# dronefreak/CABiNet

Measured on NVIDIA B200. Metric: images/sec at 1024x1024 (MNv3-L), higher is better.
Workload: dtype bf16

## Files before the change

cabinet_b200/_lib.py:

```python

from __future__ import annotations

import ctypes as C
import subprocess
from pathlib import Path

PKG = Path(__file__).resolve().parent
LIB_PATH = PKG / "libcabinet_b200.so"
CSRC = PKG / "csrc"

F32, BF16, F16 = 0, 1, 2
ACT_NONE, ACT_RELU, ACT_HSWISH, ACT_HSIGMOID, ACT_SIGMOID = 0, 1, 2, 3, 4

_p, _i, _ll, _f = C.c_void_p, C.c_int, C.c_longlong, C.c_float

SIGNATURES = {
    "cabinet_last_error": ([], C.c_char_p),
    "cabinet_abi_version": ([], _i),
    "cabinet_device_info": ([C.POINTER(_i)] * 3, _i),
    "cabinet_debug_flags": ([_i], _i),
    "cabinet_debug_read": ([_p, _i], _i),
    "cabinet_conv2d_simt": ([_p, _i, _ll, _ll, _ll, _ll, _ll, _p, _i, _ll, _ll, _ll, _p, _p, _ll, _p, _i, _ll, _ll,
                             _i, _i, _i, _i, _i, _i, _i, _i, _i, _i, _i, _i, _i, _f, _p], _i),
    "cabinet_conv_tc": ([_p, _ll, _i, _i, _i, _i, _p, _i, _i, _i, _i, _i, _p, _p, _ll, _p, _i, _ll, _i, _i, _i, _p], _i),
    "cabinet_conv_tc_dt": ([_p, _ll, _i, _i, _i, _i, _p, _i, _i, _i, _i, _i, _p, _p, _ll, _p, _i, _ll, _i, _i, _i, _i, _p],
                           _i),
    "cabinet_conv_tc_view": ([_p, _ll, _i, _i, _i, _i, _p, _i, _i, _i, _i, _p, _p, _ll, _i, _i, _ll, _ll, _ll, _p], _i),
    "cabinet_conv_tc_view_dt": ([_p, _ll, _i, _i, _i, _i, _p, _i, _i, _i, _i, _p, _p, _ll, _i, _i, _ll, _ll, _ll, _i, _p], _i),
    "cabinet_conv_tc_se": ([_p, _ll, _i, _i, _i, _i, _p, _i, _p, _i, _i, _i, _i, _i, _p, _p, _ll, _p, _i, _ll, _i, _i, _i,
                            _p], _i),
    "cabinet_conv_tc_split_act": ([_p, _ll, _i, _i, _i, _i, _p, _i, _i, _i, _i, _i, _p, _p, _i, _ll, _i, _i, _i, _i, _p], _i),
    "cabinet_conv_tc_imgw": ([_p, _ll, _i, _i, _i, _i, _p, _ll, _i, _i, _i, _i, _i, _p, _p, _ll, _p, _i, _ll, _i, _i, _i,
                              _p], _i),
    "cabinet_conv_tc_imgw_dt": ([_p, _ll, _i, _i, _i, _i, _p, _ll, _i, _i, _i, _i, _i, _p, _p, _ll, _p, _i, _ll, _i, _i, _i,
                                 _i, _p], _i),
    "cabinet_conv_tc_up": ([_p, _ll, _i, _i, _i, _i, _p, _i, _i, _i, _i, _i, _p, _p, _i, _i, _p, _ll, _i, _i, _i, _p], _i),
    "cabinet_gate_scale_weights": ([_p, _i, _f, _p, _p, _p, _p, _i, _i, _i, _p, _p, _i, _i, _i, _i, _i, _p], _i),
    "cabinet_scale_weights": ([_p, _p, _p, _i, _i, _i, _i, _i, _i, _p], _i),
    "cabinet_stem_tc": ([_p, _i, _i, _i, _p, _p, _p, _ll, _p, _ll, _i, _i, _p], _i),
    "cabinet_stem_tc2": ([_p, _i, _i, _i, _p, _p, _ll, _p, _ll, _i, _i, _p], _i),
    "cabinet_dwconv": ([_p, _ll, _p, _p, _p, _ll, _i, _i, _i, _i, _i, _i, _i, _i, _i, _i, _p, _p], _i),
    "cabinet_dwconv_tma": ([_p, _ll, _p, _p, _p, _ll, _i, _i, _i, _i, _i, _i, _i, _i, _i, _p, _p], _i),
    "cabinet_dwconv_tma_dt": ([_p, _ll, _p, _p, _p, _ll, _i, _i, _i, _i, _i, _i, _i, _i, _i, _p, _i, _p], _i),
    "cabinet_mbconv_noexpand_fused": ([_p, _ll, _p, _p, _p, _p, _p, _ll, _i, _i, _i, _i, _i, _p], _i),
    "cabinet_mbconv_fused": ([_p, _ll, _i, _i, _i, _i, _p, _p, _i, _i, _i, _i, _i, _p, _p, _i, _i, _p, _ll, _i, _i, _p,
                              _p], _i),
    "cabinet_mbconv_t": ([_p, _ll, _i, _i, _i, _i, _p, _p, _i, _i, _i, _i, _i, _p, _p, _i, _i, _p, _ll, _i, _i, _p, _p,
                          _p], _i),
    "cabinet_expand_sums": ([_p, _ll, _i, _i, _i, _i, _p, _p, _i, _i, _i, _i, _p, _p], _i),
    "cabinet_gate_mlp": ([_p, _f, _p, _p, _p, _p, _p, _i, _i, _i, _i, _p], _i),
    "cabinet_gate_fc": ([_p, _f, _p, _p, _p, _i, _i, _i, _i, _i, _p], _i),
    "cabinet_scale_act": ([_p, _ll, _i, _p, _i, _ll, _i, _i, _i, _p], _i),
    "cabinet_psp_pool": ([_p, _ll, _i, _p, _i, _i, _i, _i, _p, _ll, _p], _i),
    "cabinet_psp_concat": ([_p, _ll, _p, _p, _ll, _i, _i, _i, _i, _i, _p], _i),
    "cabinet_softmax_rows": ([_p, _p, _i, _ll, _i, _p], _i),
    "cabinet_attention_tc": ([_p, _ll, _p, _ll, _p, _ll, _p, _p, _ll, _i, _i, _i, _f, _p], _i),
    "cabinet_cab_combine": ([_p, _p, _p, _p, _ll, _p, _i, _ll, _i, _p], _i),
    "cabinet_channel_sum": ([_p, _ll, _i, _i, _ll, _i, _p, _p, _ll, _p], _i),
    "cabinet_bilinear_nhwc": ([_p, _ll, _i, _p, _ll, _i, _i, _i, _i, _i, _i, _i, _p], _i),
    "cabinet_upsample_logits_nchw": ([_p, _i, _i, _i, _i, _p, _i, _i, _i, _p], _i),
    "cabinet_upsample_argmax": ([_p, _i, _i, _i, _i, _p, _i, _i, _p, _i, _i, _p, _p], _i),
    "cabinet_normalize_u8": ([_p, _p, _i, _i, _i, _f, _f, _f, _f, _f, _f, _p], _i),
    "cabinet_confusion_hist": ([_p, _i, _p, _i, _ll, _i, _i, _p, _p], _i),
    "cabinet_upsample_softmax_accum": ([_p, _p, _i, _i, _i, _i, _i, _i, _p, _ll, _ll, _ll, _i, _i, _i, _i, _p, _p, _f,
                                        _p], _i),
    "cabinet_prob_resize_accum": ([_p, _i, _i, _i, _i, _i, _i, _i, _i, _p, _i, _i, _p], _i),
    "cabinet_argmax_hist_nchw": ([_p, _i, _i, _ll, _p, _p, _i, _i, _p, _p], _i),
    "cabinet_ohem_workspace_bytes": ([], _ll),
    "cabinet_train_scratch_floats": ([_ll, _i, _i], _ll),
    "cabinet_pack_conv_weight": ([_p, _i, _i, _i, _i, _p, _i, _i, _i, _i, _p], _i),
    "cabinet_pack_conv_weight_parity": ([_p, _i, _i, _i, _i, _i, _i, _i, _i, _i, _p, _i, _i, _p], _i),
    "cabinet_pack_conv_weight_parity_dt": ([_p, _i, _i, _i, _i, _i, _i, _i, _i, _i, _p, _i, _i, _i, _p], _i),
    "cabinet_pack_dw_weight": ([_p, _i, _i, _i, _p, _p], _i),
    "cabinet_im2col_nchw": ([_p, _i, _i, _i, _i, _i, _i, _i, _p, _ll, _p], _i),
    "cabinet_im2col_nchw_dt": ([_p, _i, _i, _i, _i, _i, _i, _i, _p, _ll, _i, _p], _i),
    "cabinet_embed_filter": ([_p, _i, _i, _i, _i, _p, _ll, _i, _p], _i),
    "cabinet_bn_train_stats": ([_p, _ll, _i, _ll, _i, _p, _p, _f, _f, _p, _p, _p, _p, _p], _i),
    "cabinet_affine_act": ([_p, _ll, _i, _p, _p, _p, _f, _p, _ll, _p, _ll, _i, _ll, _ll, _i, _i, _p], _i),
    "cabinet_bn_train_backward": ([_p, _ll, _p, _ll, _i, _p, _i, _p, _p, _p, _ll, _ll, _i, _i, _p, _p], _i),
    "cabinet_bn_frozen_stats": ([_p, _p, _p, _p, _f, _i, _p, _p], _i),
    "cabinet_bn_frozen_backward": ([_p, _ll, _p, _ll, _i, _p, _i, _p, _p, _p, _ll, _ll, _i, _i, _p, _p], _i),
    "cabinet_stem_dgrad": ([_p, _ll, _p, _ll, _i, _p, _p, _p, _i, _i, _i, _i, _i, _p], _i),
    "cabinet_gate_scale_backward": ([_p, _ll, _p, _ll, _i, _p, _f, _i, _p, _i, _ll, _i, _p, _p], _i),
    "cabinet_gate_apply_backward": ([_p, _ll, _p, _ll, _i, _p, _f, _p, _f, _i, _p, _ll, _i, _ll, _i, _i, _p], _i),
    "cabinet_gate_mlp_backward": ([_p, _f, _p, _p, _p, _p, _p, _i, _i, _i, _i, _p, _p, _p, _p, _p, _p, _p], _i),
    "cabinet_col_sum": ([_p, _ll, _i, _ll, _i, _p, _i, _p, _p], _i),
    "cabinet_conv_dgrad": ([_p, _ll, _i, _p, _i, _ll, _ll, _p, _ll, _i, _i, _i, _i, _i, _i, _i, _i, _i, _i, _i, _i, _p], _i),
    "cabinet_conv_wgrad_scratch_floats": ([_i, _i, _i, _i, _i, _i, _i], _ll),
    "cabinet_conv_wgrad": ([_p, _ll, _i, _p, _i, _ll, _ll, _ll, _ll, _p, _i, _i, _i, _i, _i, _i, _i, _i, _i, _i, _i, _p,
                            _p], _i),
    "cabinet_conv_wgrad_tc_scratch_floats": ([_i, _i, _i, _i, _i, _i, _i, _i, _i], _ll),
    "cabinet_conv_wgrad_tc": ([_p, _ll, _p, _ll, _p, _i, _i, _i, _i, _i, _i, _i, _i, _i, _p, _p], _i),
    "cabinet_conv_wgrad_tc_dt": ([_p, _ll, _p, _ll, _p, _i, _i, _i, _i, _i, _i, _i, _i, _i, _p, _i, _p], _i),
# ... 57 lines not shown
```

cabinet_b200/engine.py:

```python

from __future__ import annotations

import math
from dataclasses import dataclass
from typing import Optional

import torch

from . import _lib
from ._lib import ACT_HSIGMOID, ACT_HSWISH, ACT_NONE, ACT_RELU, ACT_SIGMOID, BF16, F16, F32, check
from .constants import BN_EPS


_DTYPE_CODES = {torch.float32: F32, torch.bfloat16: BF16, torch.float16: F16}


def dtype_code(dtype: torch.dtype) -> int:
    code = _DTYPE_CODES.get(dtype)
    if code is None:
        raise TypeError(f"cabinet_b200 kernels take float32, bfloat16 or float16 tensors, got {dtype}")
    return code


@dataclass
# ... 75 lines not shown

    def __init__(self, w1, b1, w2, b2, gate):
        f = lambda t: None if t is None else _host(t).reshape(t.shape[0], -1).contiguous()
        self.w1, self.w2 = f(w1), f(w2)
        self.b1 = None if b1 is None else _host(b1).contiguous()
        self.b2 = None if b2 is None else _host(b2).contiguous()
        self.cmid, self.c = self.w1.shape
        self.gate = gate


_LAYER_TYPES = {c.__name__: c for c in (ConvLayer, DwLayer, GateLayer)}


def _to_plain(o):
    if type(o).__name__ in _LAYER_TYPES:
        return {"__layer__": type(o).__name__, "vars": {k: _to_plain(v) for k, v in vars(o).items()}}
    if isinstance(o, dict):
        return {k: _to_plain(v) for k, v in o.items()}
    if isinstance(o, (list, tuple)):
        return type(o)(_to_plain(v) for v in o)
    return o


def _map_tensors(o, fn):
    if isinstance(o, torch.Tensor):
        return fn(o)
    if type(o).__name__ in _LAYER_TYPES:
        for k, v in vars(o).items():
            setattr(o, k, _map_tensors(v, fn))
        return o
    if isinstance(o, dict):
        return {k: _map_tensors(v, fn) for k, v in o.items()}
    if isinstance(o, (list, tuple)):
        return type(o)(_map_tensors(v, fn) for v in o)
    return o


def _from_plain(o):
    if isinstance(o, dict):
        if "__layer__" in o:
            obj = object.__new__(_LAYER_TYPES[o["__layer__"]])
            obj.__dict__.update({k: _from_plain(v) for k, v in o["vars"].items()})
            return obj
        return {k: _from_plain(v) for k, v in o.items()}
    if isinstance(o, (list, tuple)):
        return type(o)(_from_plain(v) for v in o)
    return o


def _out_size(n, k, s, p):
    return (n + 2 * p - k) // s + 1


class Engine:
    PACKED_ATTRS = ("stem", "blocks", "last", "stem_tc", "sb1", "sb2", "sb3", "sb4", "conva", "to_q", "to_k", "to_v",
                    "psp_k", "psp_v", "proj_out", "local", "gamma", "convb", "b1", "b4", "key_ch", "qkv", "ffm_blk",
                    "ffm_gate", "head_conv", "head_out", "ffm_sb", "low_fold", "stem_tc2")

    def __init__(self, model, precision: str = "bf16", packed: Optional[dict] = None):
        if precision not in ("bf16", "fp32"):
            raise ValueError(f"precision must be 'bf16' or 'fp32', got {precision!r}")
        p0 = next(model.parameters())
        if not p0.is_cuda:
            raise RuntimeError("cabinet_b200 engine needs the model on a CUDA device (no CPU path)")
        self.lib = _lib.load()
        self.dev = p0.device
        self.precision = precision
        self.tdt = torch.bfloat16 if precision == "bf16" else torch.float32
        self.dt = BF16 if precision == "bf16" else F32
        self.n_classes = model.n_classes
        self.stamp = None
        self.launches = 0
        self.use_tc = precision == "bf16"
        self.debug = False
        self.stages = {}
        self.trace, self.trace_filter = None, None
        self.fuse_mbconv = True
        self.se_from_sums = True
        self.use_stem2 = True
        self.t_small_s2 = False
        self.t_k5s2 = True
        self.use_mbconv_t = True
        self.fold_se_relu = True
        self.fold_ffm = True
        self.fold_low_up = False
        self.reverse_layers = frozenset()
        self.fuse_se = False
        self.fuse_se_blocks = frozenset({"mobile.f12", "mobile.f13"})
        self.use_cuda_graph = False
        self.sub_batch = 0
        self._graphs = {}
        self._pool = None
        self._graph_seen = {}
        self.dual_stream = False
        self._side = None
        self._scratch = []
        self.branch_overlap = True
        self._branch_streams, self._branch_events = [], {}
        self.sb_overlap = False
        if packed is not None:
            missing = [a for a in self.PACKED_ATTRS if a not in packed]
            if missing:
                raise ValueError(f"packed weights lack {missing}")
            for a in self.PACKED_ATTRS:
                setattr(self, a, _from_plain(packed[a]))
            self.gamma = model.ab.a2block.gamma.detach().float().contiguous()
        else:
            with torch.no_grad():
                self._pack(model)
                for a in self.PACKED_ATTRS:
                    setattr(self, a, _map_tensors(getattr(self, a), lambda t: t.to(self.dev)))

    def packed_state(self) -> dict:
        return {a: _to_plain(getattr(self, a)) for a in self.PACKED_ATTRS}

    def _pack(self, m):
        wd = self.tdt
        f32 = torch.float32
        mob = m.mobile
        self.stem = ConvLayer(mob.features[0][0], mob.features[0][1], ACT_HSWISH, f32, "mobile.stem")
        self.blocks = []
        for bi, blk in enumerate(list(mob.features)[1:], 1):
            s, c = blk.spec, blk.conv
            act = ACT_HSWISH if s["hs"] else ACT_RELU
            e = dict(spec=s, act=act)
            if s["expand"]:
                e["pw1"] = ConvLayer(c[0], c[1], act, wd, f"mobile.f{bi}.expand")
                e["dw"] = DwLayer(c[3], c[4], ACT_NONE if s["se"] else act, f"mobile.f{bi}.dw")
                se, pw2, bn2 = c[5], c[7], c[8]
                if self.precision == "bf16":
                    dwl, kk, nc = e["dw"], e["dw"].k ** 2, -(-e["dw"].c // 64)
                    aux = torch.zeros((nc * 64, kk + 2), dtype=f32, device=dwl.w.device)
# ... 1 lines not shown
                    aux[: dwl.c, kk + 1] = dwl.b
                    e["aux"] = aux.view(nc, 64, kk + 2).permute(0, 2, 1).contiguous()
                    p1 = e["pw1"]
                    if p1.cin % 8 == 0 and p1.cin % 64 <= 56 and p1.cin <= 248:
                        wb = torch.zeros((-(-p1.cout // 16) * 16, (p1.cin // 64 + 1) * 64), dtype=f32, device=dwl.w.device)
                        wb[: p1.cout, : p1.cin] = p1.tc[: p1.cout, 0, : p1.cin].float()
                        hi = p1.b.to(torch.bfloat16).float()
                        wb[: p1.cout, p1.cin], wb[: p1.cout, p1.cin + 1] = hi, p1.b - hi
                        e["w1b"] = wb.to(torch.bfloat16).contiguous()
                        ch = 64 if dwl.c <= 64 else 128
                        nct = 1 if dwl.c <= 64 else -(-dwl.c // 128)
                        flat = torch.zeros((nct * ch, wb.shape[1]), dtype=f32, device=dwl.w.device)
                        flat[: dwl.c] = wb[: dwl.c]
                        e["w1t"] = (flat.view(nct, ch, -1).repeat(1, 128 // ch, 1).reshape(nct * 128, -1)
                                    .to(torch.bfloat16).contiguous())
                        fa = torch.zeros((nct * ch, kk + 1), dtype=f32, device=dwl.w.device)
                        fa[: dwl.c, :kk] = dwl.w.t()
                        fa[: dwl.c, kk] = dwl.b
                        e["auxt"] = fa.view(nct, ch, kk + 1).repeat(1, 128 // ch, 1).permute(0, 2, 1).contiguous()
            else:
                e["dw"] = DwLayer(c[0], c[1], act, f"mobile.f{bi}.dw")
                se, pw2, bn2 = c[3], c[4], c[5]
            if s["se"]:
                e["se"] = GateLayer(se.fc[0].weight, se.fc[0].bias, se.fc[2].weight, se.fc[2].bias, ACT_HSIGMOID)
            e["pw2"] = ConvLayer(pw2, bn2, ACT_NONE, wd, f"mobile.f{bi}.project")
            if (not s["expand"] and not s["se"] and s["identity"] and s["k"] == 3 and s["exp"] in (8, 16, 32)
                    and self.precision == "bf16"):
                w2, b2 = _fold(pw2.weight, pw2.bias, bn2)
                e["fused_pw"] = (w2.reshape(w2.shape[0], -1).contiguous(), b2.contiguous())
            self.blocks.append(e)
        self.last = ConvLayer(mob.conv[0], mob.conv[1], ACT_HSWISH, wd, "mobile.conv")

        sb = m.sb
        self.stem_tc = self.stem_tc2 = None
        if self.precision == "bf16":
            w7, b7 = _fold(sb.conv1.conv.weight, None, sb.conv1.bn)
            w3, b3 = _fold(mob.features[0][0].weight, None, mob.features[0][1])
            pk = torch.zeros((80, 3, 7, 8), dtype=torch.float32, device=w7.device)
            pk[:64, :, :, 1:8] = w7
            pk[64:, :, 2:5, 3:6] = w3
            self.stem_tc = (pk.reshape(80, 168).contiguous(), torch.cat([b7, b3]).contiguous())
            wk = torch.zeros((80, 192), dtype=torch.float32, device=w7.device)
            wk[:, :168] = self.stem_tc[0]
            bias = self.stem_tc[1]
            b_hi = bias.to(torch.bfloat16).float()
            wk[:, 168], wk[:, 169] = b_hi, bias - b_hi
            self.stem_tc = (wk.to(torch.bfloat16).contiguous(), bias)
            wn = torch.zeros((80, 7, 8, 4), dtype=torch.float32, device=w7.device)
            wn[..., :3] = pk.permute(0, 2, 3, 1)
            wn[:, 3, 4, 3], wn[:, 3, 5, 3] = b_hi, bias - b_hi
            self.stem_tc2 = wn.view(80, 7, 2, 2, 8).permute(1, 2, 3, 0, 4).contiguous().to(torch.bfloat16)
        self.sb1 = ConvLayer(sb.conv1.conv, sb.conv1.bn, ACT_RELU, f32, "sb.conv1")
        self.sb2 = ConvLayer(sb.conv2.conv, sb.conv2.bn, ACT_RELU, wd, "sb.conv2")
        self.sb3 = ConvLayer(sb.conv3.conv, sb.conv3.bn, ACT_RELU, wd, "sb.conv3")
        self.sb4 = ConvLayer(sb.conv_out.conv, sb.conv_out.bn, ACT_RELU, wd, "sb.conv_out")

        ab, ga = m.ab, m.ab.a2block.global_attn
        self.conva = ConvLayer(ab.conva[0], ab.conva[1], ACT_RELU, wd, "ab.conva")
        self.to_q = ConvLayer(ga.to_query[0], ga.to_query[1], ACT_RELU, wd, "cab.to_query")
        self.to_k = ConvLayer(ga.to_key[0], ga.to_key[1], ACT_RELU, wd, "cab.to_key")
        self.to_v = ConvLayer(ga.to_value, None, ACT_NONE, wd, "cab.to_value")
        self.psp_k = ConvLayer(ga.psp_key.project, None, ACT_NONE, wd, "cab.psp_key")
        self.psp_v = ConvLayer(ga.psp_value.project, None, ACT_NONE, wd, "cab.psp_value")
        self.proj_out = ConvLayer(ga.project_out, None, ACT_NONE, wd, "cab.project_out")
        self.local = [DwLayer(d.block[0], d.block[1], ACT_RELU, f"cab.local{i}")
                      for i, d in enumerate(ab.a2block.local_attn.refine)]
        self.gamma = _host(ab.a2block.gamma).contiguous()
        self.convb = ConvLayer(ab.convb, None, ACT_NONE, wd, "ab.convb")
        self.b1 = ConvLayer(ab.b1, ab.b2, ACT_RELU, wd, "ab.b1")
        self.b4 = ConvLayer(ab.b4, None, ACT_NONE, wd, "ab.b4")
        self.key_ch = self.to_k.cout
        self.qkv = None
        if (self.precision == "bf16" and all(L.tc is not None and L.kh == 1 for L in (self.to_q, self.to_k, self.to_v))
                and self.to_q.cout == self.to_k.cout == self.to_v.cout and self.to_q.cout % 16 == 0):
            self.qkv = (torch.cat([L.tc[: L.cout] for L in (self.to_q, self.to_k, self.to_v)], 0).contiguous(),
                        torch.cat([self.to_q.b, self.to_k.b, self.to_v.b]).contiguous())

        ffm = m.ffm
        self.ffm_blk = ConvLayer(ffm.convblk.conv, ffm.convblk.bn, ACT_RELU, wd, "ffm.convblk")
        self.ffm_gate = GateLayer(ffm.conv1.weight, None, ffm.conv2.weight, None, ACT_SIGMOID)
        self.ffm_sb = self.low_fold = None
        if self.precision == "bf16" and ffm.convblk.conv.kernel_size == (1, 1) and ab.convb.kernel_size == (1, 1):
            wf, bf_ = _fold(ffm.convblk.conv.weight, ffm.convblk.conv.bias, ffm.convblk.bn)
            n_sb = sb.conv_out.conv.out_channels
            w_low = wf[:, n_sb:, 0, 0].double()
            wb, bb = _fold(ab.convb.weight, ab.convb.bias, None)
            self.ffm_sb = ConvLayer(None, None, ACT_RELU, wd, "ffm.convblk", folded=(wf[:, :n_sb].contiguous(), bf_, 1, 0))
            self.low_fold = ConvLayer(None, None, ACT_NONE, wd, "ab.convb*ffm.low",
                                      folded=((w_low @ wb[:, :, 0, 0].double()).float()[:, :, None, None].contiguous(),
                                              (w_low @ bb.double()).float(), 1, 0))
        self.head_conv = ConvLayer(m.conv_out.conv.conv, m.conv_out.conv.bn, ACT_RELU, wd, "conv_out.conv")
        self.head_out = ConvLayer(m.conv_out.conv_out, None, ACT_NONE, wd, "conv_out.conv_out")

    @property
    def stream(self):
        return torch.cuda.current_stream(self.dev).cuda_stream

    def _run(self, kernel: str, layer: str, nbytes: int, flops: int, fn, *args):
        nbytes, fused_bytes = nbytes if isinstance(nbytes, tuple) else (nbytes, nbytes)
        tr = self.trace
        if tr is not None and (self.trace_filter is None or kernel in self.trace_filter):
            e0, e1 = torch.cuda.Event(enable_timing=True), torch.cuda.Event(enable_timing=True)
            e0.record()
            rc = fn(*args)
            e1.record()
            tr.append((kernel, layer, nbytes, flops, e0, e1, fused_bytes))
# ... 220 lines not shown
        cat = self.new(x.N, x.H, x.W, 5 * x.C)
        self._run("psp_concat", L.name, 0, 0, self.lib.cabinet_psp_concat, x.ptr, x.ld, pooled.data_ptr(), cat.ptr,
                  cat.ld, x.dt, x.N, x.H, x.W, x.C, self.stream)
        return self.conv(cat, L)

    def attention(self, q: Map, k: Map, v: Map) -> Map:
        N, Lq, d = q.N, q.H * q.W, q.C
        es = q.t.element_size()
        ctx = self.new(q.N, q.H, q.W, d)
        if self.use_tc and d == 128 and q.dt == BF16 and all(m.ld % 8 == 0 and m.off % 8 == 0 for m in (q, k, v)):
            vt = torch.empty((N, d, -(-Lq // 8) * 8), dtype=torch.bfloat16, device=self.dev)
            self._run("attention_tc", "cab.attention", 4 * N * Lq * d * es, 4 * N * Lq * Lq * d,
                      self.lib.cabinet_attention_tc, q.ptr, q.ld, k.ptr, k.ld, v.ptr, v.ld, vt.data_ptr(), ctx.ptr,
                      ctx.ld, N, Lq, d, float(d) ** -0.5, self.stream)
            self.launches += 1
            return ctx
        s = torch.empty((N, Lq, Lq), dtype=torch.float32, device=self.dev)
        self._run("conv2d_simt", "cab.qk", 2 * N * Lq * d * es, 2 * N * Lq * Lq * d, self.lib.cabinet_conv2d_simt,
                  q.ptr, q.dt, 0, 0, q.ld, 1, Lq * q.ld, k.ptr, k.dt, k.ld, 1, Lq * k.ld, None, None, 0,
                  s.data_ptr(), F32, Lq, Lq * Lq, N, 1, 1, Lq, d, Lq, 1, 1, 1, 0, 1, Lq, ACT_NONE, float(d) ** -0.5,
                  self.stream)
        p = torch.empty((N, Lq, Lq), dtype=self.tdt, device=self.dev)
        self._run("softmax_rows", "cab.softmax", 0, 0, self.lib.cabinet_softmax_rows, s.data_ptr(), p.data_ptr(),
                  self.dt, N * Lq, Lq, self.stream)
        self._run("conv2d_simt", "cab.pv", 2 * N * Lq * d * es, 2 * N * Lq * Lq * d, self.lib.cabinet_conv2d_simt,
                  p.data_ptr(), self.dt, 0, 0, Lq, 1, Lq * Lq, v.ptr, v.dt, 1, v.ld, Lq * v.ld, None, None, 0,
                  ctx.ptr, ctx.dt, ctx.ld, Lq * ctx.ld, N, 1, 1, Lq, Lq, d, 1, 1, 1, 0, 1, Lq, ACT_NONE, 1.0,
                  self.stream)
        return ctx

    def bilinear(self, x: Map, out: Map, name: str):
        nbytes = x.N * x.C * (x.H * x.W * x.t.element_size() + out.H * out.W * out.t.element_size())
        self._run("bilinear_nhwc", name, nbytes, 0, self.lib.cabinet_bilinear_nhwc, x.ptr, x.ld, x.dt, out.ptr, out.ld,
                  out.dt, x.N, x.H, x.W, x.C, out.H, out.W, self.stream)

    def _trunk(self, x: torch.Tensor, need_aux: bool = True):
        if x.dtype != torch.float32 or not x.is_contiguous():
            x = x.float().contiguous()
        if x.device != self.dev:
            raise RuntimeError(f"input on {x.device}, model on {self.dev}")
        N, _, H, W = x.shape
        self.launches = 0
        dev, C = self.dev, self.n_classes
        n_se = sum(1 for b in self.blocks if "se" in b)
        kc = self.key_ch
        n_gap, n_psp, n_ffm = (2 * n_se + 1) * N * 1024, 128 + N * (110 + 256 * kc), 128 + N * 64 * 256
        zeros_all = torch.zeros(n_gap + 2 * n_psp + n_ffm, dtype=torch.float32, device=dev)
        gap_all = zeros_all[:n_gap].view(2 * n_se + 1, N * 1024)
        self._scratch = [zeros_all[n_gap + i * n_psp: n_gap + (i + 1) * n_psp] for i in range(2)]
        ffm_scratch = zeros_all[n_gap + 2 * n_psp:]
        self.launches += 1

        fused_stems = self.use_tc and self.stem_tc is not None and W % 4 == 0
        if fused_stems:
            OH2, OW2 = (H - 1) // 2 + 1, (W - 1) // 2 + 1
            s1, f0 = self.new(N, OH2, OW2, 64), self.new(N, OH2, OW2, 16)
            nbytes = x.numel() * 4 + (s1.t.numel() + f0.t.numel()) * 2 + 80 * 192 * 2
            if self.use_stem2 and self.stem_tc2 is not None:
                self._run("stem_tc", "sb.conv1+mobile.stem", nbytes, 2 * N * OH2 * OW2 * (64 * 147 + 16 * 27),
                          self.lib.cabinet_stem_tc2, x.data_ptr(), N, H, W, self.stem_tc2.data_ptr(), s1.ptr, s1.ld,
                          f0.ptr, f0.ld, OH2, OW2, self.stream)
            else:
                self._run("stem_tc", "sb.conv1+mobile.stem", nbytes, 2 * N * OH2 * OW2 * (64 * 147 + 16 * 27),
                          self.lib.cabinet_stem_tc, x.data_ptr(), N, H, W, self.stem_tc[0].data_ptr(),
                          self.stem_tc[1].data_ptr(), s1.ptr, s1.ld, f0.ptr, f0.ld, OH2, OW2, self.stream)
        else:
            s1 = self.conv(None, self.sb1, nchw_input=x)
        H8, W8 = _out_size(_out_size(s1.H, 3, 2, 1), 3, 2, 1), _out_size(_out_size(s1.W, 3, 2, 1), 3, 2, 1)
        fold_low = (self.fold_low_up and self.use_tc and not self.debug and self.ffm_sb is not None
                    and self.ffm_sb.tc is not None and self.low_fold.tc is not None and self.sb4.cout == self.ffm_sb.cin)
        cat_ffm = self.new(N, H8, W8, self.sb4.cout if fold_low else 128 + 256)
        if self.sb_overlap:
            with self._branch(2) as joined:
                s2 = self.conv(s1, self.sb2)
                s3 = self.conv(s2, self.sb3)
                self.conv(s3, self.sb4, out=cat_ffm.slice(0, 128))
                joined(s1.t)
        else:
            s2 = self.conv(s1, self.sb2)
            s3 = self.conv(s2, self.sb3)
            self.conv(s3, self.sb4, out=cat_ffm.slice(0, 128))
        assert (s3.H, s3.W) == (H8, W8)

        f = f0 if fused_stems else self.conv(None, self.stem, nchw_input=x)
        gi = 0
        for e in self.blocks:
            s = e["spec"]
            if "fused_pw" in e and self.use_tc and f.ld % 8 == 0 and f.off % 8 == 0:
                o = self.new(f.N, f.H, f.W, s["out"])
                dw = e["dw"]
                es = f.t.element_size()
                self._run("mbconv_noexpand_fused", dw.name.replace(".dw", ""), 2 * f.N * f.H * f.W * f.C * es,
                          2 * f.N * f.H * f.W * f.C * (9 + f.C), self.lib.cabinet_mbconv_noexpand_fused, f.ptr, f.ld,
                          dw.w.data_ptr(), dw.b.data_ptr(), e["fused_pw"][0].data_ptr(), e["fused_pw"][1].data_ptr(),
                          o.ptr, o.ld, f.N, f.H, f.W, f.C, dw.act, self.stream)
                f = o
                continue
            fuse = (s["expand"] and self.fuse_mbconv and self.use_tc and f.dt == BF16 and f.ld % 8 == 0
                    and f.off % 8 == 0 and s["exp"] % 8 == 0 and ("se" in e or s["out"] <= 160) and "w1b" in e
                    and not e.get("nofuse")
                    and not (s["k"] == 5 and s["s"] == 2 and not (self.use_mbconv_t and self.t_k5s2 and "se" in e)))
            d = None
            gap_fixed = False
            if fuse and "se" in e and self.se_from_sums and self._se_from_sums_ok(f, e):
                try:
                    f = self.se_block_one_kernel(f, e, gap_all[2 * gi:2 * gi + 2].view(-1)[: 2 * N * s["exp"]])
                    gi += 1
                    continue
                except ValueError as err:
                    if "budget" not in str(err):
                        raise
                    e["no_sums"] = True
            if fuse:
                gap = None
                if "se" in e:
                    gap, gap_fixed = gap_all[2 * gi:2 * gi + 2].view(-1)[: 2 * N * s["exp"]], True
                pw2l = e["pw2"]
                fold_se = ("se" in e and self.fold_se_relu and e["act"] == ACT_RELU and not self.debug
                           and pw2l.tc is not None and pw2l.kh == 1 and (f.H // s["s"]) * (f.W // s["s"]) % 128 == 0
                           and f.H % s["s"] == 0 and f.W % s["s"] == 0)
                try:
                    d = self.mbconv_fused(f, e, gap, ACT_RELU if fold_se else None)
                except ValueError as err:
                    if "budget" not in str(err):
                        raise
                    e["nofuse"], fuse = True, False
            if fuse and "se" not in e:
                f = d
                continue
            h = self.conv(f, e["pw1"]) if s["expand"] and not fuse else f
            if "se" in e:
                if not fuse:
# ... 296 lines not shown
```

include/cabinet_b200.h:

```cpp
#ifndef CABINET_B200_H
#define CABINET_B200_H

#include <stdint.h>

#ifdef __cplusplus
extern "C" {
#endif

#define CABINET_ABI_VERSION 2

enum { CABINET_OK = 0, CABINET_ERR_INVALID = 1, CABINET_ERR_CUDA = 2 };
enum { CABINET_F32 = 0, CABINET_BF16 = 1, CABINET_F16 = 2 };
enum {
    CABINET_ACT_NONE = 0,
    CABINET_ACT_RELU = 1,
    CABINET_ACT_HSWISH = 2,
    CABINET_ACT_HSIGMOID = 3,
    CABINET_ACT_SIGMOID = 4
};
#define CABINET_CONV_REVERSE_TILES 0x100

#define CABINET_GAP_FIXED_ONE 16777216.0f

typedef void* cabinet_stream_t;

const char* cabinet_last_error(void);
int cabinet_abi_version(void);
int cabinet_device_info(int* sm_count, int* cc_major, int* cc_minor);
int cabinet_debug_flags(int flags);
int cabinet_debug_read(long long* host_out, int n);

int cabinet_conv2d_simt(const void* x, int x_dtype, long long sxn, long long sxh, long long sxw, long long sxc,
                        long long x_batch_stride,
                        const void* w, int w_dtype, long long w_sco, long long w_sk, long long w_batch_stride,
                        const float* bias,
                        const void* res, long long ldres,
                        void* y, int y_dtype, long long ldy, long long y_batch_stride,
                        int batches, int N, int H, int W, int Cin, int Cout, int KH, int KW, int stride, int pad,
                        int OH, int OW, int act, float alpha, cabinet_stream_t stream);

int cabinet_conv_tc(const void* x, long long ldx, int N, int H, int W, int Cin, const void* w_packed, int Cout,
                    int KH, int KW, int stride, int pad, const float* bias, const void* res, long long ldres,
                    void* y, int y_dtype, long long ldy, int OH, int OW, int act, cabinet_stream_t stream);
int cabinet_conv_tc_dt(const void* x, long long ldx, int N, int H, int W, int Cin, const void* w_packed, int Cout,
                       int KH, int KW, int stride, int pad, const float* bias, const void* res, long long ldres,
                       void* y, int y_dtype, long long ldy, int OH, int OW, int act, int op_dtype, cabinet_stream_t stream);

int cabinet_conv_tc_view(const void* x, long long ldx, int N, int H, int W, int Cin, const void* w_packed, int Cout, int KH,
                         int KW, int pad, const float* bias, void* y, long long ldy, int OH, int OW, long long y_sw,
                         long long y_sh, long long y_sn, cabinet_stream_t stream);
int cabinet_conv_tc_view_dt(const void* x, long long ldx, int N, int H, int W, int Cin, const void* w_packed, int Cout, int KH,
                            int KW, int pad, const float* bias, void* y, long long ldy, int OH, int OW, long long y_sw,
                            long long y_sh, long long y_sn, int op_dtype, cabinet_stream_t stream);

int cabinet_conv_tc_se(const void* x, long long ldx, int N, int H, int W, int Cin, const float* a_scale, int a_act,
                       const void* w_packed, int Cout, int KH, int KW, int stride, int pad, const float* bias,
                       const void* res, long long ldres, void* y, int y_dtype, long long ldy, int OH, int OW, int act,
                       cabinet_stream_t stream);

int cabinet_stem_tc(const float* x, int N, int H, int W, const void* w_packed, const float* bias, void* y_sb,
                    long long ld_sb, void* y_stem, long long ld_stem, int OH, int OW, cabinet_stream_t stream);

int cabinet_stem_tc2(const float* x, int N, int H, int W, const void* w_packed2, void* y_sb, long long ld_sb, void* y_stem,
                     long long ld_stem, int OH, int OW, cabinet_stream_t stream);

int cabinet_dwconv(const void* x, long long ldx, const float* w, const float* bias, void* y, long long ldy,
                   int dtype, int N, int H, int W, int C, int k, int stride, int OH, int OW, int act,
                   float* gap_sum, cabinet_stream_t stream);

int cabinet_dwconv_tma(const void* x, long long ldx, const float* w, const float* bias, void* y, long long ldy, int N,
                       int H, int W, int C, int k, int stride, int OH, int OW, int act, long long* gap_sum,
                       cabinet_stream_t stream);
int cabinet_dwconv_tma_dt(const void* x, long long ldx, const float* w, const float* bias, void* y, long long ldy, int N,
                          int H, int W, int C, int k, int stride, int OH, int OW, int act, long long* gap_sum, int op_dtype,
                          cabinet_stream_t stream);

int cabinet_mbconv_noexpand_fused(const void* x, long long ldx, const float* w_dw, const float* b_dw,
                                  const float* w_pw, const float* b_pw, void* y, long long ldy, int N, int H, int W,
                                  int C, int act, cabinet_stream_t stream);

int cabinet_conv_tc_up(const void* x, long long ldx, int N, int H, int W, int Cin, const void* w_packed, int Cout,
                       int KH, int KW, int stride, int pad, const float* bias, const float* up, int up_h, int up_w,
                       void* y, long long ldy, int OH, int OW, int act, cabinet_stream_t stream);

int cabinet_conv_tc_split_act(const void* x, long long ldx, int N, int H, int W, int Cin, const void* w_packed, int Cout,
                              int KH, int KW, int stride, int pad, const float* bias, void* y, int y_dtype, long long ldy,
                              int OH, int OW, int act, int act_cols, cabinet_stream_t stream);

int cabinet_conv_tc_imgw(const void* x, long long ldx, int N, int H, int W, int Cin, const void* w_packed_per_image,
                         long long w_image_stride, int Cout, int KH, int KW, int stride, int pad, const float* bias,
                         const void* res, long long ldres, void* y, int y_dtype, long long ldy, int OH, int OW, int act,
                         cabinet_stream_t stream);
int cabinet_conv_tc_imgw_dt(const void* x, long long ldx, int N, int H, int W, int Cin, const void* w_packed_per_image,
                            long long w_image_stride, int Cout, int KH, int KW, int stride, int pad, const float* bias,
                            const void* res, long long ldres, void* y, int y_dtype, long long ldy, int OH, int OW, int act,
                            int op_dtype, cabinet_stream_t stream);

int cabinet_scale_weights(const void* w_packed, const float* scale, void* out, int N, int rows, int taps, int cin_pad,
                          int Cin, int plus_one, cabinet_stream_t stream);

int cabinet_gate_scale_weights(const void* gap_sum, int in_fixed, float inv_hw, const float* w1, const float* b1,
                               const float* w2, const float* b2, int gate, int C, int Cmid, const void* w_packed, void* out,
                               int N, int rows, int taps, int cin_pad, int plus_one, cabinet_stream_t stream);

int cabinet_mbconv_fused(const void* x, long long ldx, int N, int H, int W, int Cin, const void* w_expand,
                         const float* aux_packed, int Cexp, int act_expand, int k, int stride, int act_dw,
                         const void* w_project, const float* b_project, int Cout, int residual, void* y, long long ldy,
                         int OH, int OW, long long* gap_sum, cabinet_stream_t stream);

int cabinet_mbconv_t(const void* x, long long ldx, int N, int H, int W, int Cin, const void* w_expand_t, const float* aux_t,
                     int Cexp, int act_expand, int k, int stride, int act_dw, const void* w_project,
                     const float* b_project, int Cout, int residual, void* y, long long ldy, int OH, int OW,
                     long long* gap_sum, const float* se_scale, cabinet_stream_t stream);

int cabinet_expand_sums(const void* x, long long ldx, int N, int H, int W, int Cin, const void* w_expand_t,
                        const float* aux_t, int Cexp, int act_expand, int k, int nsplit, long long* gap_sum,
                        cabinet_stream_t stream);
// ... 167 lines not shown
```

Baseline: 6308.

## Fuse stem and spatial-branch conv1 with sb.conv2 into one warp-specialized tcgen05 kernel

Adds a persistent, warp-specialized kernel that computes the 7x7 sb.conv1 and the mobile stem via UMMA, keeps the sb.conv1 rows in shared memory, and then runs the stride-2 3x3 sb.conv2 directly from those rows into TMEM. This avoids writing the full-resolution 64-channel sb.conv1 activation to HBM and reading it back, and removes one launch. It adds a complex mbarrier pipeline with halo handling across strips. It only applies when sb_overlap is off and the width constraints hold.

```diff
diff --git a/cabinet_b200/_lib.py b/cabinet_b200/_lib.py
--- a/cabinet_b200/_lib.py
+++ b/cabinet_b200/_lib.py
@@ -39,6 +39,7 @@
     "cabinet_scale_weights": ([_p, _p, _p, _i, _i, _i, _i, _i, _i, _p], _i),
     "cabinet_stem_tc": ([_p, _i, _i, _i, _p, _p, _p, _ll, _p, _ll, _i, _i, _p], _i),
     "cabinet_stem_tc2": ([_p, _i, _i, _i, _p, _p, _ll, _p, _ll, _i, _i, _p], _i),
+    "cabinet_stem_sb2": ([_p, _i, _i, _i, _p, _p, _p, _ll, _p, _ll, _i, _i, _p], _i),
     "cabinet_dwconv": ([_p, _ll, _p, _p, _p, _ll, _i, _i, _i, _i, _i, _i, _i, _i, _i, _i, _p, _p], _i),
     "cabinet_dwconv_tma": ([_p, _ll, _p, _p, _p, _ll, _i, _i, _i, _i, _i, _i, _i, _i, _i, _p, _p], _i),
     "cabinet_dwconv_tma_dt": ([_p, _ll, _p, _p, _p, _ll, _i, _i, _i, _i, _i, _i, _i, _i, _i, _p, _i, _p], _i),
diff --git a/cabinet_b200/csrc/stem_sb2.cu b/cabinet_b200/csrc/stem_sb2.cu
--- /dev/null
+++ b/cabinet_b200/csrc/stem_sb2.cu
@@ -0,0 +1,394 @@
+#include <stdlib.h>
+
+#include "tc_common.cuh"
+
+namespace {
+
+constexpr int STRIP = 128;
+constexpr int MAX_R = 16;
+constexpr int DEFAULT_R = 8;
+constexpr int NR = 10;
+constexpr int IN_PX = 520;
+constexpr int PITCHI = IN_PX * 8;
+constexpr int GS_E = STRIP * 16;
+constexpr int GS_O = (STRIP + 1) * 16;
+constexpr int PLANE_E = 8 * GS_E;
+constexpr int ROWBUF = PLANE_E + 8 * GS_O;
+constexpr int W1_MMA_BYTES = 2 * 10 * 128;
+constexpr int W1_BYTES = 14 * W1_MMA_BYTES;
+constexpr int W2_MMA_BYTES = 2 * 8 * 128;
+constexpr int W2_BYTES = 36 * W2_MMA_BYTES;
+constexpr int OFF_W2 = 36864;
+constexpr int OFF_ROW = OFF_W2 + W2_BYTES;
+constexpr int OFF_IN = OFF_ROW + 2 * ROWBUF;
+constexpr int OFF_HALO = OFF_IN + NR * PITCHI;
+constexpr int SMEM_BYTES = OFF_HALO + (2 * MAX_R + 1) * 128 + 1024;
+constexpr int CONV_WARPS = 6;
+constexpr int EPI1_WARP0 = 2 + CONV_WARPS, EPI2_WARP0 = EPI1_WARP0 + 4;
+constexpr int NUM_THREADS = 32 * (EPI2_WARP0 + 4);
+constexpr int C1_SLOTS = 3, C2_COL0 = 384;
+
+struct SbParams {
+    const float* x;
+    const void* w;
+    const float* bias2;
+    bf16* y2;
+    bf16* yst;
+    long long ld2, ldst;
+    int N, H, W, OH1, OW1, OH2, OW2;
+    int R, nseg, nstrips, num_units;
+};
+
+struct Unit {
+    int n, r0, nr;
+};
+__device__ __forceinline__ Unit decode_unit(const SbParams& p, int u) {
+    Unit w;
+    w.n = u / p.nseg;
+    w.r0 = (u - w.n * p.nseg) * p.R;
+    w.nr = min(p.R, p.OH2 - w.r0);
+    return w;
+}
+
+__device__ __forceinline__ uint64_t make_desc_nosw(uint32_t smem_addr, uint32_t lbo, uint32_t sbo) {
+    uint64_t d = 0;
+    d |= static_cast<uint64_t>((smem_addr & 0x3FFFF) >> 4);
+    d |= static_cast<uint64_t>(lbo >> 4) << 16;
+    d |= static_cast<uint64_t>(sbo >> 4) << 32;
+    d |= static_cast<uint64_t>(1) << 46;
+    return d;
+}
+
+__device__ __forceinline__ uint32_t pack2(float lo, float hi) {
+    __nv_bfloat162 h = __floats2bfloat162_rn(lo, hi);
+    return *reinterpret_cast<uint32_t*>(&h);
+}
+
+__device__ __forceinline__ void stg128(void* p, const uint4& v) {
+    asm volatile("st.global.v4.u32 [%0], {%1, %2, %3, %4};" ::"l"(p), "r"(v.x), "r"(v.y), "r"(v.z), "r"(v.w) : "memory");
+}
+
+__global__ void __launch_bounds__(NUM_THREADS, 1) stem_sb2_kernel(const SbParams p) {
+    extern __shared__ uint8_t smem_raw[];
+    __shared__ __align__(8) uint64_t w_bar, in_full[NR], in_empty[NR], c1_full[C1_SLOTS], c1_empty[C1_SLOTS],
+        row_ready[2], c2_full[2], c2_empty[2];
+    __shared__ uint32_t tmem_base_smem;
+    __shared__ __align__(16) float s_bias2[64];
+
+    uint8_t* smem = reinterpret_cast<uint8_t*>((reinterpret_cast<uintptr_t>(smem_raw) + 1023) & ~uintptr_t(1023));
+    const uint32_t sW1 = tc::smem_u32(smem), sW2 = sW1 + OFF_W2, sRow = sW1 + OFF_ROW, sIn = sW1 + OFF_IN,
+                   sHalo = sW1 + OFF_HALO;
+    const int warp = threadIdx.x >> 5, lane = threadIdx.x & 31;
+
+    if (threadIdx.x < 64) s_bias2[threadIdx.x] = __ldg(p.bias2 + threadIdx.x);
+    if (threadIdx.x == 0) {
+        tc::mbar_init(&w_bar, 1);
+        for (int s = 0; s < NR; ++s) {
+            tc::mbar_init(&in_full[s], 2);
+            tc::mbar_init(&in_empty[s], 1);
+        }
+        for (int s = 0; s < C1_SLOTS; ++s) {
+            tc::mbar_init(&c1_full[s], 1);
+            tc::mbar_init(&c1_empty[s], 4);
+        }
+        for (int s = 0; s < 2; ++s) {
+            tc::mbar_init(&row_ready[s], 4);
+            tc::mbar_init(&c2_full[s], 1);
+            tc::mbar_init(&c2_empty[s], 4);
+        }
+        tc::mbar_fence_init();
+        tc::fence_proxy_async();
+    }
+    if (warp == 1) tc::tmem_alloc(&tmem_base_smem, 512);
+    tc::tc_fence_before();
+    __syncthreads();
+    tc::tc_fence_after();
+    const uint32_t tmem = tmem_base_smem;
+
+    if (warp == 0) {
+        if (lane == 0) {
+            tc::mbar_expect_tx(&w_bar, W1_BYTES + W2_BYTES);
+            asm volatile("cp.async.bulk.shared::cluster.global.mbarrier::complete_tx::bytes [%0], [%1], %2, [%3];" ::"r"(sW1),
+                         "l"(reinterpret_cast<uint64_t>(p.w)), "r"(W1_BYTES), "r"(tc::smem_u32(&w_bar))
+                         : "memory");
+            asm volatile("cp.async.bulk.shared::cluster.global.mbarrier::complete_tx::bytes [%0], [%1], %2, [%3];" ::"r"(sW2),
+                         "l"(reinterpret_cast<uint64_t>(p.w) + W1_BYTES), "r"(W2_BYTES), "r"(tc::smem_u32(&w_bar))
+                         : "memory");
+        }
+        __syncwarp();
+    } else if (warp == 1) {
+        const uint32_t leader = tc::elect_one();
+        const uint32_t id1 = tc::make_idesc_bf16(128, 80), id2 = tc::make_idesc_bf16(128, 64);
+        tc::mbar_wait(&w_bar, 0);
+        int tile_it = 0, item = 0, c2_it = 0, in_base = 0;
+        int pend_item = -1, pend_jr = 0, pend_nr = 0;
+        auto pieces = [&](int it, int jr, int nr) {
+            const int buf = it & 1;
+            tc::mbar_wait(&row_ready[buf], (it >> 1) & 1);
+            tc::tc_fence_after();
+            const uint32_t rb = sRow + buf * ROWBUF;
+            auto piece = [&](int ky) {
+                const int slot = c2_it & 1;
+                if (ky == 0) {
+                    tc::mbar_wait(&c2_empty[slot], ((c2_it >> 1) & 1) ^ 1);
+                    tc::tc_fence_after();
+                }
+                const uint32_t d = tmem + C2_COL0 + slot * 64;
+#pragma unroll
+                for (int kx = 0; kx < 3; ++kx) {
+                    const uint32_t gs = kx == 1 ? GS_E : GS_O;
+                    const uint32_t a0 = rb + (kx == 1 ? 0 : PLANE_E) + (kx == 2 ? 16 : 0);
+#pragma unroll
+                    for (int q = 0; q < 4; ++q) {
+                        const uint64_t a_desc = make_desc_nosw(a0 + q * 2 * gs, gs, 128);
+                        const uint64_t b_desc = make_desc_nosw(sW2 + ((ky * 3 + kx) * 4 + q) * W2_MMA_BYTES, 1024, 128);
+                        tc::umma_bf16_if(leader, d, a_desc, b_desc, id2, (ky | kx | q) ? 1u : 0u);
+                    }
+                }
+                if (ky == 2) {
+                    tc::umma_commit_if(leader, &c2_full[slot]);
+                    ++c2_it;
+                }
+            };
+            if (jr & 1) {
+                piece(1);
+            } else {
+                if (jr >= 2) piece(2);
+                if (jr < 2 * nr) piece(0);
+            }
+        };
+        for (int u = blockIdx.x; u < p.num_units; u += gridDim.x) {
+            const Unit un = decode_unit(p, u);
+            for (int s = 0; s < p.nstrips; ++s) {
+                for (int jr = 0; jr <= 2 * un.nr; ++jr, ++item) {
+                    for (int ky = 0; ky < 7; ++ky) {
+                        const int seq = in_base + 2 * jr + ky;
+                        tc::mbar_wait(&in_full[seq % NR], (seq / NR) & 1);
+                    }
+                    tc::tc_fence_after();
+#pragma unroll 1
+                    for (int t = 0; t < 2; ++t, ++tile_it) {
+                        const int slot = tile_it % C1_SLOTS;
+                        tc::mbar_wait(&c1_empty[slot], ((tile_it / C1_SLOTS) & 1) ^ 1);
+                        tc::tc_fence_after();
+                        const uint32_t d = tmem + slot * 128;
+#pragma unroll
+                        for (int j = 0; j < 14; ++j) {
+                            const int seq = in_base + 2 * jr + (j >> 1);
+                            const uint64_t a_desc =
+                                make_desc_nosw(sIn + (seq % NR) * PITCHI + t * 2048 + (j & 1) * 32, 16, 128);
+                            const uint64_t w_desc = make_desc_nosw(sW1 + j * W1_MMA_BYTES, 10 * 128, 128);
+                            tc::umma_bf16_if(leader, d, a_desc, w_desc, id1, j ? 1u : 0u);
+                        }
+                        tc::umma_commit_if(leader, &c1_full[slot]);
+                    }
+                    const int nfree = jr < 2 * un.nr ? 2 : 7;
+                    for (int k = 0; k < nfree; ++k) tc::umma_commit_if(leader, &in_empty[(in_base + 2 * jr + k) % NR]);
+                    if (pend_item >= 0) pieces(pend_item, pend_jr, pend_nr);
+                    pend_item = item; pend_jr = jr; pend_nr = un.nr;
+                }
+                in_base += 4 * un.nr + 7;
+            }
+        }
+        if (pend_item >= 0) pieces(pend_item, pend_jr, pend_nr);
+        __syncwarp();
+    } else if (warp < EPI1_WARP0) {
+        const int cw = warp - 2, pair = cw >> 1, ct = (cw & 1) * 32 + lane;
+        const long long plane = static_cast<long long>(p.H) * p.W;
+        int seq = 0;
+        for (int u = blockIdx.x; u < p.num_units; u += gridDim.x) {
+            const Unit un = decode_unit(p, u);
+            const float* xn = p.x + static_cast<long long>(un.n) * 3 * plane;
+            for (int s = 0; s < p.nstrips; ++s) {
+                const int col0 = 4 * s * STRIP - 4;
+                for (int t = 0; t < 4 * un.nr + 7; ++t, ++seq) {
+                    if (seq % (CONV_WARPS / 2) != pair) continue;
+                    const int y = 4 * un.r0 - 5 + t;
+                    const int slot = seq % NR;
+                    tc::mbar_wait(&in_empty[slot], ((seq / NR) & 1) ^ 1);
+                    const bool rowok = y >= 0 && y < p.H;
+                    const float* xr = xn + static_cast<long long>(rowok ? y : 0) * p.W;
+                    constexpr int K = (IN_PX + 63) / 64;
+                    float f[K][3];
+#pragma unroll
+                    for (int k = 0; k < K; ++k) {
+                        const int col = col0 + ct + 64 * k;
+                        const bool ok = rowok && ct + 64 * k < IN_PX && col >= 0 && col < p.W;
+#pragma unroll
+                        for (int c = 0; c < 3; ++c) f[k][c] = ok ? __ldg(xr + c * plane + col) : 0.f;
+                    }
+                    const uint32_t rowa = sIn + slot * PITCHI;
+#pragma unroll
+                    for (int k = 0; k < K; ++k) {
+                        const int i = ct + 64 * k;
+                        if (i < IN_PX)
+                            asm volatile("st.shared.v2.u32 [%0], {%1, %2};" ::"r"(rowa + i * 8), "r"(pack2(f[k][0], f[k][1])),
+                                         "r"(pack2(f[k][2], 1.0f))
+                                         : "memory");
+                    }
+                    tc::fence_proxy_async();
+                    __syncwarp();
+                    if (lane == 0) tc::mbar_arrive(&in_full[slot]);
+                }
+            }
+        }
+    } else if (warp < EPI2_WARP0) {
+        const int q = warp & 3, m = q * 32 + lane;
+        int tile_it = 0, item = 0;
+        for (int u = blockIdx.x; u < p.num_units; u += gridDim.x) {
+            const Unit un = decode_unit(p, u);
+            for (int s = 0; s < p.nstrips; ++s) {
+                for (int jr = 0; jr <= 2 * un.nr; ++jr, ++item) {
+                    const int rho = 2 * un.r0 - 1 + jr;
+                    const bool rowok = rho >= 0 && rho < p.OH1;
+                    const bool own = jr >= 1 && rowok;
+                    const uint32_t rb = sRow + (item & 1) * ROWBUF;
+#pragma unroll 1
+                    for (int t = 0; t < 2; ++t, ++tile_it) {
+                        const int slot = tile_it % C1_SLOTS;
+                        tc::mbar_wait(&c1_full[slot], (tile_it / C1_SLOTS) & 1);
+                        tc::tc_fence_after();
+                        const uint32_t taddr = tmem + slot * 128 + (static_cast<uint32_t>(q * 32) << 16);
+                        uint32_t a0[32], a1[32], a2[16];
+                        tc::tmem_ld32(taddr, a0);
+                        tc::tmem_ld32(taddr + 32, a1);
+                        tc::tmem_ld16(taddr + 64, a2);
+                        tc::tmem_ld_wait();
+                        tc::tc_fence_before();
+                        __syncwarp();
+                        if (lane == 0) tc::mbar_arrive(&c1_empty[slot]);
+                        const int idx = t * 128 + m;
+                        const bool odd = idx & 1;
+                        const uint32_t pb = rb + (odd ? PLANE_E + ((idx + 1) >> 1) * 16 : (idx >> 1) * 16);
+                        const uint32_t gs = odd ? GS_O : GS_E;
+                        const bool keep_halo = t == 1 && m == 127;
+#pragma unroll
+                        for (int g = 0; g < 8; ++g) {
+                            uint32_t w[4];
+#pragma unroll
+                            for (int j = 0; j < 4; ++j) {
+                                const float lo = __uint_as_float(g < 4 ? a0[8 * g + 2 * j] : a1[8 * (g - 4) + 2 * j]);
+                                const float hi = __uint_as_float(g < 4 ? a0[8 * g + 2 * j + 1] : a1[8 * (g - 4) + 2 * j + 1]);
+                                asm("cvt.rn.relu.bf16x2.f32 %0, %1, %2;" : "=r"(w[j]) : "f"(hi), "f"(lo));
+                            }
+                            const uint4 v = rowok ? make_uint4(w[0], w[1], w[2], w[3]) : make_uint4(0, 0, 0, 0);
+                            tc::sts128(pb + g * gs, v);
+                            if (keep_halo) tc::sts128(sHalo + jr * 128 + g * 16, v);
+                        }
+                        if (t == 0 && m == 0) {
+#pragma unroll
+                            for (int g = 0; g < 8; ++g) {
+                                const uint4 v = s > 0 ? tc::lds128(sHalo + jr * 128 + g * 16) : make_uint4(0, 0, 0, 0);
+                                tc::sts128(rb + PLANE_E + g * GS_O, v);
+                            }
+                        }
+                        const int col = 2 * s * STRIP + idx;
+                        if (own && col < p.OW1) {
+                            bf16* yp = p.yst + ((static_cast<long long>(un.n) * p.OH1 + rho) * p.OW1 + col) * p.ldst;
+#pragma unroll
+                            for (int g = 0; g < 2; ++g) {
+                                float v[8];
+#pragma unroll
+                                for (int j = 0; j < 8; ++j) {
+                                    const float tt = __uint_as_float(a2[8 * g + j]);
+                                    v[j] = tt * __saturatef(fmaf(tt, 1.f / 6.f, 0.5f));
+                                }
+                                Vec16<bf16> o;
+                                o.pack(v);
+                                stg128(yp + 8 * g, o.raw);
+                            }
+                        }
+                        if (t == 0) tc::named_bar_sync(1, 128);
+                    }
+                    tc::fence_proxy_async();
+                    __syncwarp();
+                    if (lane == 0) tc::mbar_arrive(&row_ready[item & 1]);
+                }
+            }
+        }
+    } else {
+        const int q = warp & 3, m = q * 32 + lane;
+        int c2_it = 0;
+        for (int u = blockIdx.x; u < p.num_units; u += gridDim.x) {
+            const Unit un = decode_unit(p, u);
+            for (int s = 0; s < p.nstrips; ++s) {
+                const int ox = s * STRIP + m;
+                for (int r = un.r0; r < un.r0 + un.nr; ++r, ++c2_it) {
+                    const int slot = c2_it & 1;
+                    tc::mbar_wait(&c2_full[slot], (c2_it >> 1) & 1);
+                    tc::tc_fence_after();
+                    const uint32_t taddr = tmem + C2_COL0 + slot * 64 + (static_cast<uint32_t>(q * 32) << 16);
+                    uint32_t a[64];
+#pragma unroll
+                    for (int c = 0; c < 4; ++c) tc::tmem_ld16(taddr + c * 16, a + 16 * c);
+                    tc::tmem_ld_wait();
+                    tc::tc_fence_before();
+                    __syncwarp();
+                    if (lane == 0) tc::mbar_arrive(&c2_empty[slot]);
+                    if (ox < p.OW2) {
+                        bf16* yp = p.y2 + ((static_cast<long long>(un.n) * p.OH2 + r) * p.OW2 + ox) * p.ld2;
+#pragma unroll
+                        for (int g = 0; g < 8; ++g) {
+                            uint32_t w[4];
+#pragma unroll
+                            for (int j = 0; j < 4; ++j) {
+                                const float lo = __uint_as_float(a[8 * g + 2 * j]) + s_bias2[8 * g + 2 * j];
+                                const float hi = __uint_as_float(a[8 * g + 2 * j + 1]) + s_bias2[8 * g + 2 * j + 1];
+                                asm("cvt.rn.relu.bf16x2.f32 %0, %1, %2;" : "=r"(w[j]) : "f"(hi), "f"(lo));
+                            }
+                            stg128(yp + 8 * g, make_uint4(w[0], w[1], w[2], w[3]));
+                        }
+                    }
+                }
+            }
+        }
+    }
+    tc::tc_fence_before();
+    __syncthreads();
+    if (warp == 1) {
+        tc::tc_fence_after();
+        tc::tmem_dealloc(tmem, 512);
+    }
+}
+
+int g_attr_set = 0;
+
+}
+
+extern "C" int cabinet_stem_sb2(const float* x, int N, int H, int W, const void* w_packed, const float* bias2, void* y_sb2,
+                                long long ld_sb2, void* y_stem, long long ld_stem, int OH2, int OW2,
+                                cabinet_stream_t stream) {
+    CAB_REQUIRE(x && w_packed && bias2 && y_sb2 && y_stem, "stem_sb2: null pointer");
+    CAB_REQUIRE(N >= 0 && H > 0 && W > 0 && W % 4 == 0, "stem_sb2: W must be a multiple of 4");
+    CAB_REQUIRE(W / 4 >= STRIP, "stem_sb2: the sb.conv2 map must be at least %d columns wide (W >= %d)", STRIP, 4 * STRIP);
+    const int OH1 = (H - 1) / 2 + 1, OW1 = (W - 1) / 2 + 1;
+    CAB_REQUIRE(OH2 == (OH1 - 1) / 2 + 1 && OW2 == (OW1 - 1) / 2 + 1, "stem_sb2: inconsistent output size");
+    CAB_REQUIRE(ld_sb2 >= 64 && ld_sb2 % 8 == 0 && ld_stem >= 16 && ld_stem % 8 == 0 &&
+                    (reinterpret_cast<uintptr_t>(y_sb2) & 15) == 0 && (reinterpret_cast<uintptr_t>(y_stem) & 15) == 0 &&
+                    (reinterpret_cast<uintptr_t>(x) & 15) == 0 && (reinterpret_cast<uintptr_t>(w_packed) & 15) == 0 &&
+                    (reinterpret_cast<uintptr_t>(bias2) & 3) == 0,
+                "stem_sb2: alignment");
+    if (N == 0) return CABINET_OK;
+    SbParams p;
+    p.x = x; p.w = w_packed; p.bias2 = bias2;
+    p.y2 = static_cast<bf16*>(y_sb2); p.yst = static_cast<bf16*>(y_stem); p.ld2 = ld_sb2; p.ldst = ld_stem;
+    p.N = N; p.H = H; p.W = W; p.OH1 = OH1; p.OW1 = OW1; p.OH2 = OH2; p.OW2 = OW2;
+    static const int rows_env = getenv("CAB_SB2_ROWS") ? atoi(getenv("CAB_SB2_ROWS")) : 0;
+    p.R = rows_env >= 1 && rows_env <= MAX_R ? rows_env : DEFAULT_R;
+    p.nseg = (OH2 + p.R - 1) / p.R;
+    p.nstrips = (OW2 + STRIP - 1) / STRIP;
+    const long long nu = static_cast<long long>(N) * p.nseg;
+    CAB_REQUIRE(nu < (1LL << 31), "stem_sb2: too many work units");
+    p.num_units = static_cast<int>(nu);
+    if (!g_attr_set) {
+        CAB_CUDA(cudaFuncSetAttribute(stem_sb2_kernel, cudaFuncAttributeMaxDynamicSharedMemorySize, SMEM_BYTES));
+        g_attr_set = 1;
+    }
+    int dev = 0, sms = 148;
+    CAB_CUDA(cudaGetDevice(&dev));
+    CAB_CUDA(cudaDeviceGetAttribute(&sms, cudaDevAttrMultiProcessorCount, dev));
+    const int grid = static_cast<int>(std::min<long long>(nu, sms));
+    stem_sb2_kernel<<<grid, NUM_THREADS, SMEM_BYTES, static_cast<cudaStream_t>(stream)>>>(p);
+    CAB_LAUNCH_CHECK();
+    return CABINET_OK;
+}
diff --git a/cabinet_b200/engine.py b/cabinet_b200/engine.py
--- a/cabinet_b200/engine.py
+++ b/cabinet_b200/engine.py
@@ -151,10 +151,14 @@
     return (n + 2 * p - k) // s + 1
 
 
+def stem_sb2_supported(H, W):
+    return H > 0 and W % 4 == 0 and W // 4 >= 128
+
+
 class Engine:
     PACKED_ATTRS = ("stem", "blocks", "last", "stem_tc", "sb1", "sb2", "sb3", "sb4", "conva", "to_q", "to_k", "to_v",
                     "psp_k", "psp_v", "proj_out", "local", "gamma", "convb", "b1", "b4", "key_ch", "qkv", "ffm_blk",
-                    "ffm_gate", "head_conv", "head_out", "ffm_sb", "low_fold", "stem_tc2")
+                    "ffm_gate", "head_conv", "head_out", "ffm_sb", "low_fold", "stem_tc2", "stem_sb2")
 
     def __init__(self, model, precision: str = "bf16", packed: Optional[dict] = None):
         if precision not in ("bf16", "fp32"):
@@ -177,6 +181,7 @@
         self.fuse_mbconv = True
         self.se_from_sums = True
         self.use_stem2 = True
+        self.fuse_stem_sb2 = True
         self.t_small_s2 = False
         self.t_k5s2 = True
         self.use_mbconv_t = True
@@ -284,6 +289,10 @@
             self.stem_tc2 = wn.view(80, 7, 2, 2, 8).permute(1, 2, 3, 0, 4).contiguous().to(torch.bfloat16)
         self.sb1 = ConvLayer(sb.conv1.conv, sb.conv1.bn, ACT_RELU, f32, "sb.conv1")
         self.sb2 = ConvLayer(sb.conv2.conv, sb.conv2.bn, ACT_RELU, wd, "sb.conv2")
+        self.stem_sb2 = None
+        if self.stem_tc2 is not None and self.sb2.tc is not None and tuple(self.sb2.tc.shape) == (64, 9, 64):
+            w2 = self.sb2.tc.view(64, 9, 4, 2, 8).permute(1, 2, 3, 0, 4).reshape(-1)
+            self.stem_sb2 = torch.cat([self.stem_tc2.reshape(-1), w2]).contiguous()
         self.sb3 = ConvLayer(sb.conv3.conv, sb.conv3.bn, ACT_RELU, wd, "sb.conv3")
         self.sb4 = ConvLayer(sb.conv_out.conv, sb.conv_out.bn, ACT_RELU, wd, "sb.conv_out")
 
@@ -610,7 +619,19 @@
         self.launches += 1
 
         fused_stems = self.use_tc and self.stem_tc is not None and W % 4 == 0
-        if fused_stems:
+        fused_sb2 = (fused_stems and self.use_stem2 and self.fuse_stem_sb2 and self.stem_sb2 is not None
+                     and stem_sb2_supported(H, W) and not self.sb_overlap and "sb.conv2" not in self.reverse_layers)
+        s2 = None
+        if fused_sb2:
+            OH2, OW2 = (H - 1) // 2 + 1, (W - 1) // 2 + 1
+            OH4, OW4 = _out_size(OH2, 3, 2, 1), _out_size(OW2, 3, 2, 1)
+            s2, f0 = self.new(N, OH4, OW4, 64), self.new(N, OH2, OW2, 16)
+            nbytes = x.numel() * 4 + (s2.t.numel() + f0.t.numel()) * 2 + self.stem_sb2.numel() * 2
+            flops = 2 * N * OH2 * OW2 * (64 * 147 + 16 * 27) + 2 * N * OH4 * OW4 * 64 * 576
+            self._run("stem_sb2", "sb.conv1+mobile.stem+sb.conv2", nbytes, flops, self.lib.cabinet_stem_sb2, x.data_ptr(),
+                      N, H, W, self.stem_sb2.data_ptr(), self.sb2.b.data_ptr(), s2.ptr, s2.ld, f0.ptr, f0.ld, OH4, OW4,
+                      self.stream)
+        elif fused_stems:
             OH2, OW2 = (H - 1) // 2 + 1, (W - 1) // 2 + 1
             s1, f0 = self.new(N, OH2, OW2, 64), self.new(N, OH2, OW2, 16)
             nbytes = x.numel() * 4 + (s1.t.numel() + f0.t.numel()) * 2 + 80 * 192 * 2
@@ -624,7 +645,10 @@
                           self.stem_tc[1].data_ptr(), s1.ptr, s1.ld, f0.ptr, f0.ld, OH2, OW2, self.stream)
         else:
             s1 = self.conv(None, self.sb1, nchw_input=x)
-        H8, W8 = _out_size(_out_size(s1.H, 3, 2, 1), 3, 2, 1), _out_size(_out_size(s1.W, 3, 2, 1), 3, 2, 1)
+        if s2 is None:
+            H8, W8 = _out_size(_out_size(s1.H, 3, 2, 1), 3, 2, 1), _out_size(_out_size(s1.W, 3, 2, 1), 3, 2, 1)
+        else:
+            H8, W8 = _out_size(s2.H, 3, 2, 1), _out_size(s2.W, 3, 2, 1)
         fold_low = (self.fold_low_up and self.use_tc and not self.debug and self.ffm_sb is not None
                     and self.ffm_sb.tc is not None and self.low_fold.tc is not None and self.sb4.cout == self.ffm_sb.cin)
         cat_ffm = self.new(N, H8, W8, self.sb4.cout if fold_low else 128 + 256)
@@ -635,7 +659,8 @@
                 self.conv(s3, self.sb4, out=cat_ffm.slice(0, 128))
                 joined(s1.t)
         else:
-            s2 = self.conv(s1, self.sb2)
+            if s2 is None:
+                s2 = self.conv(s1, self.sb2)
             s3 = self.conv(s2, self.sb3)
             self.conv(s3, self.sb4, out=cat_ffm.slice(0, 128))
         assert (s3.H, s3.W) == (H8, W8)
diff --git a/include/cabinet_b200.h b/include/cabinet_b200.h
--- a/include/cabinet_b200.h
+++ b/include/cabinet_b200.h
@@ -63,6 +63,9 @@
 
 int cabinet_stem_tc2(const float* x, int N, int H, int W, const void* w_packed2, void* y_sb, long long ld_sb, void* y_stem,
                      long long ld_stem, int OH, int OW, cabinet_stream_t stream);
+
+int cabinet_stem_sb2(const float* x, int N, int H, int W, const void* w_packed, const float* bias2, void* y_sb2,
+                     long long ld_sb2, void* y_stem, long long ld_stem, int OH2, int OW2, cabinet_stream_t stream);
 
 int cabinet_dwconv(const void* x, long long ldx, const float* w, const float* bias, void* y, long long ldy,
                    int dtype, int N, int H, int W, int C, int k, int stride, int OH, int OW, int act,
```

Measured after the change: 6451 (median of 6 runs). +2.3%, better.
